# pasensio97/SDslam

Hardware: AMD Instinct MI355X
Metric: tracked frames/sec (ORB+ImageAlign+PnP) at 640x480, 1000 kp (higher is better)
Workload: dtype u8; 1 GPU; BASELINE configs[3] at the configs[1] pyramid: 640x480, 8-level x1.2, 1000 kp; ORB extract + ImageAlign (levels 4,3,2) + SearchByProjection + PnP RANSAC (maxIts 200; iterations actually run: tracking.mean_pnp_iterations with --full); pose_solver=pnp, pyramid=8x1.2, unique_scenes=64, inputs=resident in HBM, pose_records=packed on the device every step (single GPU: no collective)

## Files before the change

include/sdslam_hip.h:

```cpp
#ifndef SDSLAM_HIP_H_
#define SDSLAM_HIP_H_

#include <stddef.h>
#include <stdint.h>

#ifdef __cplusplus
extern "C" {
#endif

#define SD_OK 0
#define SD_ERR_INVALID_ARG 1
#define SD_ERR_HIP 2
#define SD_ERR_CAPACITY 3
#define SD_ERR_NO_DEVICE 4
#define SD_FALSE 100

const char* sd_last_error(void);
int sd_device_count(void);
const char* sd_version(void);

int sd_set_option(const char* name, int value);
int sd_get_option(const char* name, int* value);
int sd_option_count(void);
const char* sd_option_name(int index);
// ... 171 lines not shown
#define SD_REFRESH_NORMAL 2
#define SD_REFRESH_SKIPPED 16
#define SD_REFRESH_NOT_RESIDENT 32
#define SD_REFRESH_TOO_MANY 64
#define SD_REFRESH_BAD_INDEX 128
int sd_track_set_observations(sd_track* h, int n_points, const int32_t* obs_off, const int32_t* obs_frame, const int32_t* obs_kp,
                              const uint8_t* obs_kf_bad, const int32_t* ref_obs, const uint8_t* point_bad);
int sd_track_refresh_points(sd_track* h, int point_row, int write_local);
int sd_track_get_refreshed(sd_track* h, uint8_t* status, int32_t* best_obs, int32_t* best_median, uint8_t* desc, double* normal,
                           float* max_dist, float* min_dist, int cap);
int sd_debug_refresh_points(int n_points, const int32_t* obs_off, const uint8_t* obs_desc, const double* obs_centre,
                            const int32_t* obs_octave, const uint8_t* obs_kf_bad, const int32_t* ref_obs, const uint8_t* point_bad,
                            const double* Xw, const float* scale_factors, int nlevels, uint8_t* status, int32_t* best_obs,
                            int32_t* best_median, uint8_t* desc, double* normal, float* max_dist, float* min_dist);

int sd_track_align(sd_track* h, int n_frames, int mode);
int sd_track_match(sd_track* h, int n_frames, float th, int mono, int check_ori);
int sd_track_pnp(sd_track* h, int n_frames, double probability, int min_inliers, int max_iterations,
                 int min_set, float epsilon, float th2, int n_iterations);
int sd_track_pnp_iterate(sd_track* h, int n_frames, int n_iterations);
int sd_track_set_matches(sd_track* h, int frame0, int n_frames, const int32_t* cur_match, int cap);

int sd_track_get_align(sd_track* h, int frame0, int n_frames, double* Tcur_cm, double* error,
                       int32_t* ok, int32_t* iters, double* chi2);
int sd_track_get_matches(sd_track* h, int frame0, int n_frames, int32_t* cur_match, int cap,
                         int32_t* n_matches);
int sd_track_get_pnp(sd_track* h, int frame0, int n_frames, float* Tcw_rowmajor, uint8_t* inliers,
                     int cap, int32_t* info8);
int sd_debug_pnp_prof(unsigned long long* out32, int reset);
int sd_debug_align_prof(unsigned long long* out16, int reset);
int sd_debug_sel_prof(unsigned long long* out64, int reset);
int sd_debug_epnp(int n, const double* Xw, const double* uv, double fx, double fy, double cx, double cy,
                  double* R9, double* t3, double* reproj_err);
int sd_track_debug_read(sd_track* h, int which, int frame, void* out, size_t bytes);
int sd_track_debug_features_in_area(sd_track* h, int frame, float x, float y, float r, int min_level, int max_level,
                                    int32_t* indices, int cap, int32_t* n_out, int32_t* grid_counts);
int sd_track_pack_records(sd_track* h, int n_frames, int source, void* d_records);

int sd_track_set_map_ids(sd_track* h, int frame0, int n_frames, int which, const int32_t* ids, int cap);
int sd_track_advance(sd_track* h, int n_frames, int source);
int sd_track_set_prior(sd_track* h, int frame0, int n_frames, const double* T_cm, int relative);
int sd_track_get_last(sd_track* h, int frame0, int n_frames, int32_t* n_last, uint8_t* valid, double* Xw, uint8_t* desc, int32_t* octave,
                      float* angle, int32_t* obs, int32_t* ids);
int sd_track_get_extractors(sd_track* h, sd_orb** cur, sd_orb** ref);
int sd_track_close_points(sd_track* h, int n_frames, int source, float th_depth);
int sd_track_get_close_points(sd_track* h, int frame0, int n_frames, int32_t* out2);

int sd_track_motion_predict(sd_track* h, int n_frames, double dt);
int sd_track_motion_update(sd_track* h, int n_frames, int source);
int sd_track_motion_restart(sd_track* h, int frame0, int n_frames);
int sd_track_get_motion(sd_track* h, int frame0, int n_frames, double* X6, double* Pdiag6, int32_t* started, double* it_time,
                        double* E_cm, double* last_pose_cm);
int sd_track_set_motion(sd_track* h, int frame0, int n_frames, const double* X6, const double* Pdiag6, const int32_t* started,
                        const double* it_time);

#define SD_SENSOR_CONSTANT_VELOCITY 0
#define SD_SENSOR_IMU 1
int sd_track_set_sensor_model(sd_track* h, int model);
int sd_track_get_sensor_model(sd_track* h, int* model);
int sd_track_set_measurements(sd_track* h, int frame0, int n_frames, const double* wa6);
int sd_track_get_imu(sd_track* h, int frame0, int n_frames, double* X16, double* P256, double* gravity3, int32_t* started, double* it_time,
                     double* last_pose_cm, double* measurements6);
int sd_track_set_imu(sd_track* h, int frame0, int n_frames, const double* X16, const double* P256, const double* gravity3,
                     const int32_t* started, const double* it_time);
int sd_track_stream_fence(sd_track* h, void* hip_stream, int direction);
int sd_track_set_profiling(sd_track* h, int on);
// ... 19 lines not shown
```

sdslam_amd/capi.py:

```python
import ctypes as C
import os

import numpy as np

_HERE = os.path.dirname(os.path.abspath(__file__))
KP_DTYPE = np.dtype([("x", "<f4"), ("y", "<f4"), ("size", "<f4"), ("angle", "<f4"),
                     ("response", "<f4"), ("octave", "<i4"), ("class_id", "<i4")])
assert KP_DTYPE.itemsize == 28

SD_OK = 0


class SdError(RuntimeError):
    def __init__(self, code, msg):
        super().__init__(f"sdslam_hip status {code}: {msg}")
        self.code = code


def lib_path() -> str:
    return os.environ.get("SD_LIB") or os.path.join(_HERE, "libsdslam_hip.so")


_I, _F, _D, _Z, _P, _S = C.c_int, C.c_float, C.c_double, C.c_size_t, C.c_void_p, C.c_char_p
_PP, _PI = C.POINTER(C.c_void_p), C.POINTER(C.c_int)
# ... 71 lines not shown
    "sd_track_set_f12": (_I, [_P, _I, _I, _P]),
    "sd_track_search_for_triangulation": (_I, [_P, _I, _I, _I]),
    "sd_track_get_triangulation_matches": (_I, [_P, _I, _I, _P, _I, _P, _P, _P]),
    "sd_debug_search_for_triangulation": (_I, [_I, _I, _P, _P, _P, _P, _P, _P, _P, _P, _P, _P, _P, _P, _I, _I, _P, _P]),
    "sd_track_set_tri_depth": (_I, [_P, _I, _I, _I, _P, _I]),
    "sd_track_set_tri_median_depth": (_I, [_P, _I, _I, _P]),
    "sd_track_triangulate": (_I, [_P, _I, _I]),
    "sd_track_get_triangulated": (_I, [_P, _I, _I, _P, _P, _P, _I, _P]),
    "sd_track_get_new_points": (_I, [_P, _P, _P, _P, _P, _P, _P, _P, _P, _P, _P, _I]),
    "sd_debug_triangulate": (_I, [_I, _I, _P, _P, _P, _P, _P, _P, _P, _P, _P, _P, _P, _P, _P, _P, _I, _F, _I, _F, _P, _P, _P]),
    "sd_track_append_new_points": (_I, [_P, _I, _I, _I]),
    "sd_track_get_appended": (_I, [_P, _I, _I, _P, _P, _P]),
    "sd_track_get_local_points": (_I, [_P, _I, _P, _P, _P, _P, _P, _P, _P, _P, _P, _I]),
    "sd_track_set_fuse_scw": (_I, [_P, _I, _I, _P]),
    "sd_track_fuse": (_I, [_P, _I, _I, _I, _F, _I]),
    "sd_track_get_fuse": (_I, [_P, _I, _I, _P, _P, _I, _P]),
    "sd_debug_fuse": (_I, [_I, _P, _P, _P, _I, _P, _P, _P, _P, _P, _P, _P, _P, _I, _P, _P, _P, _I, _F, _F, _I, _I, _P, _P, _P, _P]),
    "sd_track_set_observations": (_I, [_P, _I, _P, _P, _P, _P, _P, _P]),
    "sd_track_refresh_points": (_I, [_P, _I, _I]),
    "sd_track_get_refreshed": (_I, [_P, _P, _P, _P, _P, _P, _P, _P, _I]),
    "sd_debug_refresh_points": (_I, [_I, _P, _P, _P, _P, _P, _P, _P, _P, _P, _I, _P, _P, _P, _P, _P, _P, _P]),
    "sd_track_align": (_I, [_P, _I, _I]),
    "sd_track_match": (_I, [_P, _I, _F, _I, _I]),
    "sd_track_pnp": (_I, [_P, _I, _D, _I, _I, _I, _F, _F, _I]),
    "sd_track_pnp_iterate": (_I, [_P, _I, _I]),
    "sd_track_set_matches": (_I, [_P, _I, _I, _P, _I]),
    "sd_track_get_align": (_I, [_P, _I, _I, _P, _P, _P, _P, _P]),
    "sd_track_get_matches": (_I, [_P, _I, _I, _P, _I, _P]),
    "sd_track_get_pnp": (_I, [_P, _I, _I, _P, _P, _I, _P]),
    "sd_debug_pnp_prof": (_I, [_P, _I]),
    "sd_debug_align_prof": (_I, [_P, _I]),
    "sd_debug_sel_prof": (_I, [_P, _I]),
    "sd_debug_epnp": (_I, [_I, _P, _P, _D, _D, _D, _D, _P, _P, _P]),
    "sd_track_debug_read": (_I, [_P, _I, _I, _P, _Z]),
    "sd_track_debug_features_in_area": (_I, [_P, _I, _F, _F, _F, _I, _I, _P, _I, _P, _P]),
    "sd_track_pack_records": (_I, [_P, _I, _I, _P]),
    "sd_track_set_map_ids": (_I, [_P, _I, _I, _I, _P, _I]),
    "sd_track_advance": (_I, [_P, _I, _I]),
    "sd_track_set_prior": (_I, [_P, _I, _I, _P, _I]),
    "sd_track_get_last": (_I, [_P, _I, _I, _P, _P, _P, _P, _P, _P, _P, _P]),
    "sd_track_get_extractors": (_I, [_P, _PP, _PP]),
    "sd_track_close_points": (_I, [_P, _I, _I, _F]),
    "sd_track_get_close_points": (_I, [_P, _I, _I, _P]),
    "sd_track_motion_predict": (_I, [_P, _I, _D]),
    "sd_track_motion_update": (_I, [_P, _I, _I]),
    "sd_track_motion_restart": (_I, [_P, _I, _I]),
    "sd_track_get_motion": (_I, [_P, _I, _I, _P, _P, _P, _P, _P, _P]),
    "sd_track_set_motion": (_I, [_P, _I, _I, _P, _P, _P, _P]),
    "sd_track_set_sensor_model": (_I, [_P, _I]),
    "sd_track_get_sensor_model": (_I, [_P, _PI]),
    "sd_track_set_measurements": (_I, [_P, _I, _I, _P]),
    "sd_track_get_imu": (_I, [_P, _I, _I, _P, _P, _P, _P, _P, _P, _P]),
    "sd_track_set_imu": (_I, [_P, _I, _I, _P, _P, _P, _P, _P]),
    "sd_track_stream_fence": (_I, [_P, _P, _I]),
    "sd_track_set_profiling": (_I, [_P, _I]),
    "sd_track_stage_ms": (_I, [_P, _P, _I]),
    "sd_track_set_next_map_id": (_I, [_P, _I, _I, _P]),
    "sd_track_stereo_init": (_I, [_P, _I, _I]),
    "sd_track_set_keyframe_state": (_I, [_P, _I, _I, _P]),
    "sd_track_need_keyframe": (_I, [_P, _I, _I, _I, _I, _I]),
    "sd_track_set_keyframe_flags": (_I, [_P, _I, _I, _P]),
    "sd_track_get_keyframe_flags": (_I, [_P, _I, _I, _P]),
    "sd_track_create_keyframe_points": (_I, [_P, _I, _I, _F, _I, _I]),
    "sd_track_get_created": (_I, [_P, _I, _I, _P, _P, _P, _P, _I]),
    "sd_hamming": (_I, [_P, _P]),
}
# ... 734 lines not shown
        _check(self.L.sd_track_get_keyframe_flags(self.h, frame0, n, _p(out)))
        return out

    def create_keyframe_points(self, n_frames, source, th_depth, use_flags=False, frame_id=0):
        _check(self.L.sd_track_create_keyframe_points(self.h, n_frames, int(source), float(th_depth), int(bool(use_flags)), int(frame_id)))

    def get_created(self, frame0, n, cap=None):
        cap = self.cap if cap is None else cap
        info = np.zeros((n, 4), np.int32)
        idx, ids, Xw = np.full((n, cap), -1, np.int32), np.full((n, cap), -1, np.int32), np.zeros((n, cap, 3))
        _check(self.L.sd_track_get_created(self.h, frame0, n, _p(info), _p(idx), _p(Xw), _p(ids), cap))
        return dict(mode=info[:, 0].copy(), created=info[:, 1].copy(), P=info[:, 2].copy(), candidates=info[:, 3].copy(), kp_index=idx,
                    Xw=Xw, ids=ids)

    def set_profiling(self, on=True):
        _check(self.L.sd_track_set_profiling(self.h, int(on)))

    def stage_ms(self):
        ms = np.zeros(3, np.float32)
        _check(self.L.sd_track_stage_ms(self.h, _p(ms), 3))
        return ms


def debug_epnp(Xw, uv, K):
    L = lib()
    Xw = np.ascontiguousarray(Xw, np.float64)
    uv = np.ascontiguousarray(uv, np.float64)
    R, t, e = np.zeros(9), np.zeros(3), C.c_double()
    _check(L.sd_debug_epnp(len(Xw), _p(Xw), _p(uv), float(K[0]), float(K[1]), float(K[2]), float(K[3]), _p(R), _p(t),
                           C.byref(e)))
    return R.reshape(3, 3), t, e.value


def debug_search_for_triangulation(kps1, desc1, has_mp1, uright1, kps2, desc2, has_mp2, uright2, F12, epipole, scale_factors,
                                   level_sigma2, check_ori=False):
    L = lib()
    k1, k2 = np.ascontiguousarray(kps1, KP_DTYPE), np.ascontiguousarray(kps2, KP_DTYPE)
    n1, n2 = len(k1), len(k2)
    d1, d2 = np.ascontiguousarray(desc1, np.uint8).reshape(n1, 32), np.ascontiguousarray(desc2, np.uint8).reshape(n2, 32)
    h1, h2 = np.ascontiguousarray(has_mp1, np.uint8), np.ascontiguousarray(has_mp2, np.uint8)
    u1, u2 = np.ascontiguousarray(uright1, np.float32), np.ascontiguousarray(uright2, np.float32)
    assert len(h1) == len(u1) == n1 and len(h2) == len(u2) == n2
    F, e = np.ascontiguousarray(F12, np.float64).reshape(9), np.ascontiguousarray(epipole, np.float32).reshape(2)
    sf, s2 = np.ascontiguousarray(scale_factors, np.float32), np.ascontiguousarray(level_sigma2, np.float32)
    assert len(sf) == len(s2)
    m, n = np.full(max(n1, 1), -1, np.int32), np.zeros(1, np.int32)
    _check(L.sd_debug_search_for_triangulation(n1, n2, _p(k1), _p(d1), _p(h1), _p(u1), _p(k2), _p(d2), _p(h2), _p(u2), _p(F), _p(e),
                                               _p(sf), _p(s2), len(sf), int(check_ori), _p(m), _p(n)))
    return int(n[0]), m[:n1]


def debug_triangulate(kps1_un, kps1, uright1, depth1, kps2_un, kps2, uright2, depth2, matches12, Tcw1, Tcw2, cam5, scale_factors,
                      level_sigma2, scale_factor, monocular=True, median_depth=-1.0):
    L = lib()
    k1u, k1 = np.ascontiguousarray(kps1_un, KP_DTYPE), np.ascontiguousarray(kps1, KP_DTYPE)
    k2u, k2 = np.ascontiguousarray(kps2_un, KP_DTYPE), np.ascontiguousarray(kps2, KP_DTYPE)
    n1, n2 = len(k1u), len(k2u)
    u1, z1 = np.ascontiguousarray(uright1, np.float32), np.ascontiguousarray(depth1, np.float32)
    u2, z2 = np.ascontiguousarray(uright2, np.float32), np.ascontiguousarray(depth2, np.float32)
    m = np.ascontiguousarray(matches12, np.int32)
    assert len(k1) == len(u1) == len(z1) == len(m) == n1 and len(k2) == len(u2) == len(z2) == n2
    T1, T2 = _cm(Tcw1), _cm(Tcw2)
    cam = np.ascontiguousarray(cam5, np.float32)
    sf, s2 = np.ascontiguousarray(scale_factors, np.float32), np.ascontiguousarray(level_sigma2, np.float32)
    assert len(cam) == 5 and len(sf) == len(s2)
    v, b, X = np.zeros(max(n1, 1), np.uint8), np.zeros(max(n1, 1), np.uint8), np.zeros((max(n1, 1), 3))
# ... 70 lines not shown
```

sdslam_amd/csrc/track.hip:

```cpp
#include <hip/hip_runtime.h>

#include <cmath>
#include <cstdlib>
#include <cstring>
#include <string>
#include <type_traits>
#include <vector>

#include "track_handle.h"

using namespace sd;

__global__ void k_pack_records(TrackBuffers tb, int source, int n_frames, double* __restrict__ out) {
  const int f = blockIdx.x * blockDim.x + threadIdx.x;
  if (f >= n_frames) return;
  double* r = out + (size_t)f * 20;
  if (source == 0) {
    const float* T = tb.pnp_T + (size_t)f * 16;
    for (int c = 0; c < 4; c++)
      for (int rr = 0; rr < 4; rr++) r[c * 4 + rr] = (double)T[rr * 4 + c];
  } else {
    const double* T = (source == 4 ? tb.Tcur : tb.po_T) + (size_t)f * 16;
    for (int i = 0; i < 16; i++) r[i] = T[i];
  }
// ... 755 lines not shown
}

int sd_track_get_pnp(sd_track* h, int frame0, int n_frames, float* Tcw_rowmajor, uint8_t* inliers, int cap, int32_t* info8) {
  TRACK_RANGE(h, frame0, n_frames);
  SD_REQUIRE(!inliers || cap >= h->kp_cap, SD_ERR_CAPACITY, "cap smaller than the keypoint capacity");
  hipStream_t s = h->cur->stream;
  SD_TRY(download(Tcw_rowmajor, h->tb.pnp_T, frame0, n_frames, 16, s));
  SD_TRY(download_rows(inliers, cap, h->tb.pnp_inliers, frame0, n_frames, h->kp_cap, s));
  SD_TRY(download(info8, h->tb.pnp_info, frame0, n_frames, 8, s));
  return wait_for(s);
}

int sd_debug_pnp_prof(unsigned long long* out32, int reset) {
  SD_REQUIRE(out32, SD_ERR_INVALID_ARG, "null output");
  return read_pnp_prof(out32, reset);
}

int sd_debug_sel_prof(unsigned long long* out64, int reset) {
  SD_REQUIRE(out64, SD_ERR_INVALID_ARG, "null output");
  return read_sel_prof(out64, reset);
}

int sd_debug_align_prof(unsigned long long* out16, int reset) {
  SD_REQUIRE(out16, SD_ERR_INVALID_ARG, "null output");
  return read_align_prof(out16, reset);
}

int sd_debug_epnp(int n, const double* Xw, const double* uv, double fx, double fy, double cx, double cy, double* R9, double* t3,
                  double* reproj_err) {
  SD_REQUIRE(n >= 4 && Xw && uv && R9 && t3, SD_ERR_INVALID_ARG, "bad arguments");
  return run_epnp_debug(n, Xw, uv, fx, fy, cx, cy, R9, t3, reproj_err);
}

int sd_track_debug_read(sd_track* h, int which, int frame, void* out, size_t bytes) {
  SD_REQUIRE(h && out && frame >= 0 && frame < h->max_batch, SD_ERR_INVALID_ARG, "bad arguments");
  SD_REQUIRE(which != 2 || bytes <= 15 * sizeof(double), SD_ERR_CAPACITY, "the Fuse pose of a slot is 15 doubles");
  const size_t M = (size_t)h->max_points, row = (size_t)frame * M;
  const size_t lm_bytes[5] = {M * 32, M * 24, M * 4, M * 4, M * 4};
  SD_REQUIRE(which < 3 || (which <= 7 && bytes <= lm_bytes[which - 3]), SD_ERR_CAPACITY, "unknown buffer or more bytes than a local-map row holds");
  SD_HIP_CHECK(hipSetDevice(h->device));
  SD_HIP_CHECK(hipStreamSynchronize(h->pnp_stream));
  SD_HIP_CHECK(hipStreamSynchronize(h->cur->stream));
  const void* src = which == 0   ? (const void*)(h->tb.pnp_pts + (size_t)frame * h->kp_cap * 6)
                    : which == 2 ? (const void*)(h->fu.pose + (size_t)frame * 15)
                    : which == 3 ? (const void*)(h->tb.lm_desc + row * 32)
                    : which == 4 ? (const void*)(h->tb.lm_normal + row * 3)
                    : which == 5 ? (const void*)(h->tb.lm_min + row)
                    : which == 6 ? (const void*)(h->tb.lm_max + row)
                    : which == 7 ? (const void*)(h->tb.lm_mfmax + row)
                                 : (const void*)(h->tb.pnp_kpidx + (size_t)frame * h->kp_cap);
  SD_HIP_CHECK(hipMemcpy(out, src, bytes, hipMemcpyDeviceToHost));
  return SD_OK;
}

int sd_track_debug_features_in_area(sd_track* h, int frame, float x, float y, float r, int min_level, int max_level, int32_t* indices,
                                    int cap, int32_t* n_out, int32_t* grid_counts) {
  SD_TRY(check_ready(h, frame + 1, true));
  SD_REQUIRE(frame >= 0 && indices && n_out && cap >= 0, SD_ERR_INVALID_ARG, "bad arguments");
  hipStream_t s = h->pnp_stream;
  SD_TRY(wait_inputs(h, false));
  int32_t* d = nullptr;
  const size_t n_ints = (size_t)h->kp_cap + 1 + 64 * 48;
  SD_HIP_CHECK(hipMalloc(&d, n_ints * sizeof(int32_t)));
  const int rc = launch_features_in_area(h->cur, h->tb, h->cam, frame, x, y, r, min_level, max_level, d, h->kp_cap, d + h->kp_cap, d + h->kp_cap + 1, s);
  std::vector<int32_t> host(n_ints);
  hipError_t e = hipMemcpyAsync(host.data(), d, n_ints * sizeof(int32_t), hipMemcpyDeviceToHost, s);
// ... 71 lines not shown
```

sdslam_amd/csrc/track_internal.h:

```cpp
#pragma once
#include <hip/hip_runtime.h>
#include <stdint.h>

#include "orb_internal.h"

namespace sd {

struct TrackBuffers {
  int max_points;
  int kp_cap;
  int cur_bcast;
  uint8_t* valid;
  double* Xw;
  uint8_t* mp_desc;
  int32_t* octave;
  float* angle;
  int32_t* obs;
  int32_t* n_last;
  int32_t* last_id;
  uint8_t* valid2;
  double* Xw2;
  uint8_t* mp_desc2;
  int32_t* octave2;
  float* angle2;
// ... 214 lines not shown
int launch_stereo_from_depth(const sd_orb* cur, const TrackBuffers& tb, const TrackCam& cam, const float* d_depth, int w, int h,
                             int stride_elems, size_t frame_stride_elems, int n_frames, hipStream_t s);
int launch_stereo_from_depth_typed(const sd_orb* cur, const TrackBuffers& tb, const TrackCam& cam, const void* d_depth, int u16,
                                   int convert, float scale, int w, int h, int stride_elems, size_t frame_stride_elems, int n_frames,
                                   hipStream_t s);
int launch_new_points(const sd_orb* cur, const TrackBuffers& tb, const TrackCam& cam, float inv_fx, float inv_fy, int n_frames, int mode,
                      int source, float th_depth, int use_flags, int frame_id, int min_keypoints, hipStream_t s);
int launch_need_keyframe(const TrackBuffers& tb, const int32_t* d_close, int n_frames, int rgbd, int frame_id, int min_frames,
                         int max_frames, hipStream_t s);
int launch_set_keyframe_state(const TrackBuffers& tb, const int32_t* staged, int frame0, int n_frames, hipStream_t s);
int launch_motion_init(const TrackBuffers& tb, int frame0, int n_frames, hipStream_t s);
int launch_motion_predict(const TrackBuffers& tb, int n_frames, double dt, hipStream_t s);
int launch_motion_update(const TrackBuffers& tb, int n_frames, int source, hipStream_t s);
int launch_imu_init(const TrackBuffers& tb, int frame0, int n_frames, int full, hipStream_t s);
int launch_imu_predict(const TrackBuffers& tb, int n_frames, double dt, hipStream_t s);
int launch_imu_update(const TrackBuffers& tb, int n_frames, int source, hipStream_t s);
int read_pnp_prof(unsigned long long* out32, int reset);
int read_sel_prof(unsigned long long* out64, int reset);
int read_align_prof(unsigned long long* out16, int reset);
int launch_pnp(const sd_orb* cur, const TrackBuffers& tb, const TrackCam& cam, const float* d_sigma2, const PnpParams& pp,
               int n_frames, hipStream_t s);

struct Sim3Params {
  int fix_scale, min_inliers;
  int n_iterations;
  int rand_per_frame;
  int resume;
};
int launch_sim3(const sd_orb* cur, const sd_orb* ref, const TrackBuffers& tb, const TrackCam& cam, const float* d_sigma2,
                const int32_t* d_max_its, const Sim3Params& sp, int n_frames, hipStream_t s);

int run_epnp_debug(int n, const double* Xw, const double* uv, double fx, double fy, double cx, double cy, double* R9, double* t3,
                   double* err);

}
```

sdslam_amd/csrc/track_pnp.hip:

```cpp
#include <hip/hip_runtime.h>

#include <algorithm>
#include <cfloat>
#include <cstdlib>

#include "orb_internal.h"
#include "sd_hypot.h"
#include "sd_wave.h"
#include "track_internal.h"
#include "track_pnp_lds.h"

namespace sd {

#define PNP_MAXN 2048
#define PNP_WORDS (PNP_MAXN / 64)
#define PNP_MAXSET 64

#ifdef SD_PNP_PROF
__device__ unsigned long long g_pnp_prof[32];
#define PROF_DECL long long _pt = clock64()
#define PROF(i)                                                                                       \
  do {                                                                                                \
    long long _n = clock64();                                                                         \
    if ((threadIdx.x & 63) == 0) atomicAdd(&g_pnp_prof[i], (unsigned long long)(_n - _pt));           \
    _pt = _n;                                                                                         \
  } while (0)
#else
#define PROF_DECL
#define PROF(i)
#endif

#ifndef PNP_FN
#define PNP_FN static __noinline__ __attribute__((disable_tail_calls))
#endif

typedef __attribute__((address_space(3))) double ldsd;
#define LDS_PTR(shared_array) ((ldsd*)(shared_array))
struct LArr {
  ldsd* p;
  __device__ __forceinline__ ldsd& operator[](int i) const { return p[i * PNP_CHUNK]; }
// ... 109 lines not shown
    for (int k = 0; k < m; k++) {
      double t = At[i * astep + k];
      sd += t * t;
    }
    sd = sqrt(sd);
  }
  *rng_io = rng;
  return sd;
}

template <int M, int N>
__device__ __forceinline__ void jacobi_svd_small(double (&At)[N][M], double (&Wout)[N], double (&Vt)[N][N]) {
  const double eps = DBL_EPSILON * 10, minval = DBL_MIN;
  double W[N];
#pragma unroll
  for (int i = 0; i < N; i++) {
    double sd = 0;
#pragma unroll
    for (int k = 0; k < M; k++) sd += At[i][k] * At[i][k];
    W[i] = sd;
#pragma unroll
    for (int k = 0; k < N; k++) Vt[i][k] = k == i ? 1 : 0;
  }
  for (int iter = 0; iter < 30; iter++) {
    bool changed = false;
#pragma unroll
    for (int i = 0; i < N - 1; i++) {
#pragma unroll
      for (int j = i + 1; j < N; j++) {
        double p = 0;
#pragma unroll
        for (int k = 0; k < M; k++) p += At[i][k] * At[j][k];
        if (!(fabs(p) <= eps * sqrt(W[i] * W[j]))) {
          p *= 2;
          double c, s;
          const double beta = W[i] - W[j], gamma = sdsc::hypot_glibc(p, beta);
          if (beta < 0) {
            const double delta = (gamma - beta) * 0.5;
            s = sqrt(delta / gamma);
            c = p / (gamma * s * 2);
          } else {
            c = sqrt((gamma + beta) / (gamma * 2));
            s = p / (gamma * c * 2);
          }
          double na = 0, nb = 0;
#pragma unroll
          for (int k = 0; k < M; k++) {
            const double t0 = c * At[i][k] + s * At[j][k];
            const double t1 = -s * At[i][k] + c * At[j][k];
            At[i][k] = t0;
            At[j][k] = t1;
            na += t0 * t0;
            nb += t1 * t1;
          }
          W[i] = na;
          W[j] = nb;
          changed = true;
#pragma unroll
          for (int k = 0; k < N; k++) {
            const double t0 = c * Vt[i][k] + s * Vt[j][k];
            const double t1 = -s * Vt[i][k] + c * Vt[j][k];
            Vt[i][k] = t0;
            Vt[j][k] = t1;
          }
        }
      }
    }
    if (!changed) break;
  }
#pragma unroll
  for (int i = 0; i < N; i++) {
    double sd = 0;
#pragma unroll
    for (int k = 0; k < M; k++) sd += At[i][k] * At[i][k];
    W[i] = sqrt(sd);
  }
#pragma unroll
// ... 20 lines not shown
  for (int i = 0; i < N; i++) Wout[i] = W[i];
  unsigned long long rng = 0x12345678ull;
#pragma unroll
  for (int i = 0; i < N; i++) {
    double sd = W[i];
    if (sd <= minval) {
      double tmp[N * M];
      for (int r = 0; r < N; r++)
        for (int k = 0; k < M; k++) tmp[r * M + k] = At[r][k];
      sd = jacobi_fill_row(tmp, M, M, i, &rng, sd);
#pragma unroll
      for (int k = 0; k < M; k++) At[i][k] = tmp[i * M + k];
    }
    const double s = sd > minval ? 1 / sd : 0.;
#pragma unroll
    for (int k = 0; k < M; k++) At[i][k] *= s;
  }
}

__device__ __forceinline__ bool jacobi_pair12(LMat A, int i, int j) {
  const double eps = DBL_EPSILON * 10;
  const LArr Ai = A.row(i), Aj = A.row(j);
  double ai[12], aj[12];
#pragma unroll
  for (int k = 0; k < 12; k++) {
    ai[k] = Ai[k];
    aj[k] = Aj[k];
  }
  double p = 0;
#pragma unroll
  for (int k = 0; k < 12; k++) p += ai[k] * aj[k];
  const double a = Ai[pnp_lds::kMatW], b = Aj[pnp_lds::kMatW];
  if (fabs(p) <= eps * sqrt(a * b)) return false;
  p *= 2;
  double c, s;
  const double beta = a - b, gamma = sdsc::hypot_glibc(p, beta);
  if (beta < 0) {
    const double delta = (gamma - beta) * 0.5;
    s = sqrt(delta / gamma);
    c = p / (gamma * s * 2);
  } else {
    c = sqrt((gamma + beta) / (gamma * 2));
    s = p / (gamma * c * 2);
  }
  double na = 0, nb = 0;
#pragma unroll
  for (int k = 0; k < 12; k++) {
    const double t0 = c * ai[k] + s * aj[k];
    const double t1 = -s * ai[k] + c * aj[k];
    Ai[k] = t0;
    Aj[k] = t1;
    na += t0 * t0;
    nb += t1 * t1;
  }
  Ai[pnp_lds::kMatW] = na;
  Aj[pnp_lds::kMatW] = nb;
  return true;
}

__device__ PNP_FN void jacobi_sweeps12_coop(LMat A, int g, bool act, unsigned long long group_mask) {
  if (act && g < 6)
    for (int i = g; i < 12; i += 6) {
      const LArr Ai = A.row(i);
      double sd = 0;
#pragma unroll
      for (int k = 0; k < 12; k++) {
        const double t = Ai[k];
        sd += t * t;
      }
      A.w(i) = sd;
    }
  __syncthreads();
  bool live = act;
  for (int iter = 0; iter < 30; iter++) {
    bool changed = false;
    for (int st = 1; st <= 21; st++) {
      const int i = max(0, st - 11) + g, j = st - i;
// ... 22 lines not shown
      Vt[i * 3 + j] = vt[i][j];
    }
  }
}

template <typename Ptr>
__device__ __forceinline__ void solve_svd6_n(int N, Ptr L, const int (&col)[5], const double (&b)[6], double (&x)[5]) {
  constexpr int M = 6, NM = 5;
  const double eps = DBL_EPSILON * 10, minval = DBL_MIN;
  double At[NM][M], Vt[NM][NM], W[NM];
#pragma unroll
  for (int i = 0; i < NM; i++) {
#pragma unroll
    for (int j = 0; j < M; j++) At[i][j] = i < N ? L[10 * j + col[i]] : 0.0;
    double sd = 0;
#pragma unroll
    for (int k = 0; k < M; k++) sd += At[i][k] * At[i][k];
    W[i] = sd;
#pragma unroll
    for (int k = 0; k < NM; k++) Vt[i][k] = k == i ? 1 : 0;
  }
  bool live = true;
  for (int iter = 0; iter < 30; iter++) {
    bool changed = false;
#pragma unroll
    for (int i = 0; i < NM - 1; i++) {
#pragma unroll
      for (int j = i + 1; j < NM; j++) {
        if (live && j < N) {
          double p = 0;
#pragma unroll
          for (int k = 0; k < M; k++) p += At[i][k] * At[j][k];
          if (!(fabs(p) <= eps * sqrt(W[i] * W[j]))) {
            p *= 2;
            double c, sn;
            const double beta = W[i] - W[j], gamma = sdsc::hypot_glibc(p, beta);
            if (beta < 0) {
              const double delta = (gamma - beta) * 0.5;
              sn = sqrt(delta / gamma);
              c = p / (gamma * sn * 2);
            } else {
              c = sqrt((gamma + beta) / (gamma * 2));
              sn = p / (gamma * c * 2);
            }
            double na = 0, nb = 0;
#pragma unroll
            for (int k = 0; k < M; k++) {
              const double t0 = c * At[i][k] + sn * At[j][k];
              const double t1 = -sn * At[i][k] + c * At[j][k];
              At[i][k] = t0;
              At[j][k] = t1;
              na += t0 * t0;
              nb += t1 * t1;
            }
            W[i] = na;
            W[j] = nb;
            changed = true;
#pragma unroll
            for (int k = 0; k < NM; k++) {
              const double t0 = c * Vt[i][k] + sn * Vt[j][k];
              const double t1 = -sn * Vt[i][k] + c * Vt[j][k];
              Vt[i][k] = t0;
              Vt[j][k] = t1;
            }
          }
        }
      }
    }
    live = live && changed;
    if (!__any(live)) break;
  }
#pragma unroll
  for (int i = 0; i < NM; i++) {
    double sd = 0;
#pragma unroll
    for (int k = 0; k < M; k++) sd += At[i][k] * At[i][k];
    W[i] = sqrt(sd);
// ... 431 lines not shown
    PROF(7);
    double sum2 = 0.0;
    for (int i = 0; i < n; i++) sum2 += epnp_reproj_term(Rv, tv, pws + 3 * i, us[2 * i], us[2 * i + 1], cam);
    err = sum2 / n;
    PROF(8);
  }
  return err;
}

template <int K, typename F>
__device__ __forceinline__ void ordered_sums(int n, ldsd* terms, ldsd* out, F&& term) {
  constexpr int KP = K | 1;
  const int lane = threadIdx.x & 63;
  double acc = 0;
  for (int base = 0; base < n; base += 64) {
    const int i = base + lane;
    if (i < n) {
      double tv[K];
      term(i, tv);
#pragma unroll
      for (int k = 0; k < K; k++) terms[lane * KP + k] = tv[k];
    }
    __syncthreads();
    const int cnt = min(64, n - base);
    if (lane < K) {
#pragma unroll 8
      for (int j = 0; j < cnt; j++) acc += terms[j * KP + lane];
    }
    __syncthreads();
  }
  if (lane < K) out[lane] = acc;
  __syncthreads();
}

template <typename TIn>
__device__ PNP_FN void epnp_refit_wave(int n, const TIn* pws, const TIn* us, const EpnpCam cam, ldsd* Rt_out, LMat ut, ldsd* scr) {
  const int lane = threadIdx.x & 63;
  ldsd* const terms = scr + pnp_lds::kTerms;
  ldsd* const mtm = scr + pnp_lds::kMtm;
  ldsd* const red = scr + pnp_lds::kRed;
  const LArr L{scr + pnp_lds::kRefitL};
  double cws[4][3], ci[9];
  auto PW = [&](int i, double* p) {
    p[0] = (double)pws[3 * i];
    p[1] = (double)pws[3 * i + 1];
    p[2] = (double)pws[3 * i + 2];
  };
  PROF_DECL;
  ordered_sums<3>(n, terms, red, [&](int i, double* tv) { PW(i, tv); });
  for (int j = 0; j < 3; j++) cws[0][j] = red[j] / n;
  ordered_sums<6>(n, terms, red, [&](int i, double* tv) {
    double pw[3];
    PW(i, pw);
    const double d0 = pw[0] - cws[0][0], d1 = pw[1] - cws[0][1], d2 = pw[2] - cws[0][2];
    tv[0] = d0 * d0; tv[1] = d0 * d1; tv[2] = d0 * d2;
    tv[3] = d1 * d1; tv[4] = d1 * d2; tv[5] = d2 * d2;
  });
  if (lane == 0) {
    const double pw0tpw0[9] = {red[0], red[1], red[2], red[1], red[3], red[4], red[2], red[4], red[5]};
    epnp_control_points(pw0tpw0, n, cws);
    epnp_cc_inverse(cws, ci);
    for (int i = 0; i < 9; i++) {
      red[16 + i] = cws[1 + i / 3][i % 3];
      red[32 + i] = ci[i];
    }
    for (int j = 0; j < 3; j++) red[48 + j] = cws[0][j];
// ... 46 lines not shown
          const double m2a = aa * (ca == 1 ? cam.fv : row[5]), m2b = ab * (cb == 1 ? cam.fv : row[5]);
          acc += has1 ? m1a * m1b : 0.0;
          acc += has2 ? m2a * m2b : 0.0;
        }
      }
    }
    if (mine) {
      mtm[ea * 12 + eb] = acc;
      mtm[eb * 12 + ea] = acc;
    }
  }
  __syncthreads();
  PROF(18);
  double rho[6];
  for (int i = lane; i < 144; i += 64) ut.row(i / 12)[i % 12] = mtm[i];
  __syncthreads();
  jacobi_sweeps12_coop(ut, lane, true, 0x3full);
  if (lane == 0) jacobi_finish12(ut);
  PROF(19);
  epnp_L_rho(ut, cws, L, rho, lane == 0);
  __syncthreads();
  PROF(20);
  if (lane < 3) {
    Rho6 rv;
    for (int i = 0; i < 6; i++) rv.r[i] = rho[i];
    Betas4 bt;
    epnp_betas(lane + 1, L, rv, bt);
    for (int i = 0; i < 4; i++) red[4 * lane + i] = bt.b[i];
  }
  __syncthreads();
  asm volatile("" ::: "memory");
  for (int i = 0; i < 12; i++) cws[i / 3][i % 3] = red[i < 3 ? 48 + i : 13 + i];
  for (int i = 0; i < 9; i++) ci[i] = red[32 + i];
  double betas3[3][4];
  for (int i = 0; i < 12; i++) betas3[i / 4][i % 4] = red[i];
  __syncthreads();
  PROF(22);
  double bestR[3][3], bestT[3], best_err = 0;
  for (int variant = 1; variant <= 3; variant++) {
    double ccs[4][3];
    epnp_ccs(ut, betas3[variant - 1], ccs);
    bool flip = false;
    auto PC = [&](int i, double* pc) {
      double a[4];
      AL(i, a);
      for (int j = 0; j < 3; j++) {
        const double x = a[0] * ccs[0][j] + a[1] * ccs[1][j] + a[2] * ccs[2][j] + a[3] * ccs[3][j];
        pc[j] = flip ? -x : x;
      }
    };
    {
      double pc_first[3];
      PC(0, pc_first);
      flip = pc_first[2] < 0.0;
    }
    double pc0[3], pw0[3], Rv[3][3], tv[3];
    ordered_sums<6>(n, terms, red, [&](int i, double* t6) {
      PC(i, t6);
      PW(i, t6 + 3);
    });
    for (int j = 0; j < 3; j++) {
      pc0[j] = red[j] / n;
      pw0[j] = red[3 + j] / n;
    }
    ordered_sums<9>(n, terms, red, [&](int i, double* t9) {
      double pc[3], pw[3];
      PC(i, pc);
      PW(i, pw);
      for (int j = 0; j < 3; j++) {
        t9[3 * j] = (pc[j] - pc0[j]) * (pw[0] - pw0[0]);
        t9[3 * j + 1] = (pc[j] - pc0[j]) * (pw[1] - pw0[1]);
        t9[3 * j + 2] = (pc[j] - pc0[j]) * (pw[2] - pw0[2]);
      }
    });
    if (lane == 0) {
      double abt[9];
      for (int i = 0; i < 9; i++) abt[i] = red[i];
      epnp_Rt_from_abt(abt, pc0, pw0, Rv, tv);
      for (int i = 0; i < 9; i++) red[16 + i] = Rv[i / 3][i % 3];
      for (int i = 0; i < 3; i++) red[25 + i] = tv[i];
    }
    __syncthreads();
    for (int i = 0; i < 9; i++) Rv[i / 3][i % 3] = red[16 + i];
    for (int i = 0; i < 3; i++) tv[i] = red[25 + i];
    PROF(23);
    ordered_sums<1>(n, terms, red, [&](int i, double* t1) {
      double pw[3];
      PW(i, pw);
      t1[0] = epnp_reproj_term(Rv, tv, pw, (double)us[2 * i], (double)us[2 * i + 1], cam);
    });
    const double err = red[0] / n;
    __syncthreads();
    PROF(24);
    if (variant == 1 || err < best_err) {
      best_err = err;
      for (int i = 0; i < 3; i++) {
        for (int j = 0; j < 3; j++) bestR[i][j] = Rv[i][j];
        bestT[i] = tv[i];
      }
    }
  }
  if (lane == 0) {
    for (int i = 0; i < 9; i++) Rt_out[i] = bestR[i / 3][i % 3];
    for (int i = 0; i < 3; i++) Rt_out[9 + i] = bestT[i];
    red[63] = best_err;
  }
  __syncthreads();
}

__device__ __forceinline__ bool pnp_is_inlier(const double* Rt, const float* q , const EpnpCam cam) {
  const float* p2 = q;
  const float* p3 = q + 2;
  const float maxErr = q[5];
  float Xc = (float)(Rt[0] * p3[0] + Rt[1] * p3[1] + Rt[2] * p3[2] + Rt[9]);
  float Yc = (float)(Rt[3] * p3[0] + Rt[4] * p3[1] + Rt[5] * p3[2] + Rt[10]);
  float invZc = (float)(1 / (Rt[6] * p3[0] + Rt[7] * p3[1] + Rt[8] * p3[2] + Rt[11]));
  double ue = cam.uc + cam.fu * Xc * invZc;
  double ve = cam.vc + cam.fv * Yc * invZc;
  float distX = (float)(p2[0] - ue);
  float distY = (float)(p2[1] - ve);
  float error2 = distX * distX + distY * distY;
  return error2 < maxErr;
}

template <bool kGeneral>
__global__ __launch_bounds__(64, 2) __attribute__((disable_tail_calls)) void k_pnp(const sd_keypoint* __restrict__ kps_all, const int32_t* __restrict__ nkp_all,
                                            TrackBuffers tb, TrackCam tcam, const float* __restrict__ sigma2, PnpParams pp,
                                            int n_frames) {
  __shared__ double s_work[pnp_lds::kWorkDoubles];
  __shared__ double s_Rt[PNP_CHUNK][12];
  __shared__ unsigned long long s_mask[PNP_CHUNK][PNP_WORDS];
  __shared__ unsigned long long s_best[PNP_WORDS], s_ref[PNP_WORDS];
  __shared__ int s_cnt[PNP_CHUNK];
  __shared__ double s_RtRef[12];
  __shared__ float s_bestT[12];
  __shared__ double s_scr[pnp_lds::kScrDoubles];
  __shared__ int s_modp[PNP_MAXSET], s_modv[PNP_MAXSET], s_draw[PNP_MAXSET];
  const int lane = threadIdx.x;
// ... 266 lines not shown
    for (int i = lane; i < N; i += 64)
      if ((s_ref[i >> 6] >> (i & 63)) & 1ull) inl_out[g_idx[i]] = 1;
    if (lane == 0) {
      for (int r = 0; r < 3; r++) {
        for (int c = 0; c < 3; c++) T_out[r * 4 + c] = (float)s_RtRef[r * 3 + c];
        T_out[r * 4 + 3] = (float)s_RtRef[9 + r];
      }
      T_out[12] = T_out[13] = T_out[14] = 0.f;
      T_out[15] = 1.f;
      info[0] = 1; info[1] = acc_cnt; info[2] = 0; info[3] = acc_iters; info[7] = 1;
    }
    return;
  }
  if (lane == 0) {
    info[2] = 1;
    info[3] = total;
  }
  if (best >= minInl) {
    for (int i = lane; i < N; i += 64)
      if ((s_best[i >> 6] >> (i & 63)) & 1ull) inl_out[g_idx[i]] = 1;
    if (lane == 0) {
      for (int r = 0; r < 3; r++) {
        for (int c = 0; c < 3; c++) T_out[r * 4 + c] = s_bestT[r * 3 + c];
        T_out[r * 4 + 3] = s_bestT[9 + r];
      }
      T_out[12] = T_out[13] = T_out[14] = 0.f;
      T_out[15] = 1.f;
      info[0] = 1;
      info[1] = best;
    }
  }
}

__global__ __launch_bounds__(64, 2) __attribute__((disable_tail_calls)) void k_epnp_debug(int n, const double* pws, const double* us, EpnpCam cam, double* out13) {
  __shared__ double s_work[pnp_lds::kWorkDoubles], s_scr[pnp_lds::kScrDoubles], s_Rt[12];
  const int lane = threadIdx.x;
  double e;
  if (n == 4) {
    double R[3][3], t[3];
    const int hyp = lane % PNP_CHUNK, variant = lane / PNP_CHUNK + 1;
    const bool active = hyp == 0 && variant <= 3;
    const LMat h_ut{LDS_PTR(s_work), hyp};
    const LArr h_L{LDS_PTR(s_scr) + pnp_lds::kL + hyp};
    const double err = epnp_minimal(
        active, variant,
        [&](int k, double* pw, double* u) {
          for (int j = 0; j < 3; j++) pw[j] = pws[3 * k + j];
          for (int j = 0; j < 2; j++) u[j] = us[2 * k + j];
        },
        cam, R, t, h_ut, h_L, LDS_PTR(s_scr), 1);
    const double e1 = __shfl(err, 0), e2 = __shfl(err, PNP_CHUNK), e3 = __shfl(err, 2 * PNP_CHUNK);
    int win = 1;
    e = e1;
    if (e2 < e) { win = 2; e = e2; }
    if (e3 < e) { win = 3; e = e3; }
    if (active && variant == win) {
      for (int i = 0; i < 9; i++) s_Rt[i] = R[i / 3][i % 3];
      for (int i = 0; i < 3; i++) s_Rt[9 + i] = t[i];
    }
    __syncthreads();
  } else {
    epnp_refit_wave(n, pws, us, cam, LDS_PTR(s_Rt), LMat{LDS_PTR(s_work), 0}, LDS_PTR(s_scr));
    e = s_scr[pnp_lds::kRed + 63];
  }
  if (lane == 0) {
    for (int i = 0; i < 12; i++) out13[i] = s_Rt[i];
    out13[12] = e;
  }
}

int run_epnp_debug(int n, const double* Xw, const double* uv, double fx, double fy, double cx, double cy, double* R9, double* t3,
                   double* err) {
  double *d_p = nullptr, *d_u = nullptr, *d_o = nullptr;
  SD_HIP_CHECK(hipMalloc(&d_p, sizeof(double) * 3 * n));
  SD_HIP_CHECK(hipMalloc(&d_u, sizeof(double) * 2 * n));
  SD_HIP_CHECK(hipMalloc(&d_o, sizeof(double) * 13));
  SD_HIP_CHECK(hipMemcpy(d_p, Xw, sizeof(double) * 3 * n, hipMemcpyHostToDevice));
  SD_HIP_CHECK(hipMemcpy(d_u, uv, sizeof(double) * 2 * n, hipMemcpyHostToDevice));
  EpnpCam cam = {fx, fy, cx, cy};
  hipLaunchKernelGGL(k_epnp_debug, dim3(1), dim3(64), 0, 0, n, d_p, d_u, cam, d_o);
  double out[13];
  SD_HIP_CHECK(hipMemcpy(out, d_o, sizeof(out), hipMemcpyDeviceToHost));
  for (int i = 0; i < 9; i++) R9[i] = out[i];
  for (int i = 0; i < 3; i++) t3[i] = out[9 + i];
  if (err) *err = out[12];
  (void)hipFree(d_p); (void)hipFree(d_u); (void)hipFree(d_o);
  return SD_OK;
}

int read_pnp_prof(unsigned long long* out32, int reset) {
#ifdef SD_PNP_PROF
  SD_HIP_CHECK(hipDeviceSynchronize());
  SD_HIP_CHECK(hipMemcpyFromSymbol(out32, HIP_SYMBOL(g_pnp_prof), 32 * sizeof(unsigned long long)));
  if (reset) {
    unsigned long long z[32] = {};
    SD_HIP_CHECK(hipMemcpyToSymbol(HIP_SYMBOL(g_pnp_prof), z, sizeof(z)));
  }
  return SD_OK;
#else
  set_error("library built without -DSD_PNP_PROF");
  return SD_ERR_INVALID_ARG;
#endif
}

int launch_pnp(const sd_orb* cur, const TrackBuffers& tb, const TrackCam& cam, const float* d_sigma2, const PnpParams& pp,
               int n_frames, hipStream_t s) {
  hipLaunchKernelGGL(pp.min_set == 4 ? k_pnp<false> : k_pnp<true>, dim3(n_frames), dim3(64), 0, s, keys_un(cur), cur->d_nout, tb, cam, d_sigma2, pp, n_frames);
  SD_HIP_CHECK(hipGetLastError());
  return SD_OK;
}

}
```

Measured before the change: 241,900 frames/s.

## Evaluate the three EPnP refit variants in parallel across wave lanes

Result: no change. 243,100 frames/s, median of 6 (+0.5%).

```diff
diff --git a/include/sdslam_hip.h b/include/sdslam_hip.h
--- a/include/sdslam_hip.h
+++ b/include/sdslam_hip.h
@@ -227,6 +227,8 @@
 int sd_debug_sel_prof(unsigned long long* out64, int reset);
 int sd_debug_epnp(int n, const double* Xw, const double* uv, double fx, double fy, double cx, double cy,
                   double* R9, double* t3, double* reproj_err);
+int sd_debug_epnp_variant(int n, const double* Xw, const double* uv, double fx, double fy, double cx, double cy,
+                          double* R9, double* t3, double* reproj_err, int32_t* variant2);
 int sd_track_debug_read(sd_track* h, int which, int frame, void* out, size_t bytes);
 int sd_track_debug_features_in_area(sd_track* h, int frame, float x, float y, float r, int min_level, int max_level,
                                     int32_t* indices, int cap, int32_t* n_out, int32_t* grid_counts);
diff --git a/sdslam_amd/capi.py b/sdslam_amd/capi.py
--- a/sdslam_amd/capi.py
+++ b/sdslam_amd/capi.py
@@ -127,6 +127,7 @@
     "sd_debug_align_prof": (_I, [_P, _I]),
     "sd_debug_sel_prof": (_I, [_P, _I]),
     "sd_debug_epnp": (_I, [_I, _P, _P, _D, _D, _D, _D, _P, _P, _P]),
+    "sd_debug_epnp_variant": (_I, [_I, _P, _P, _D, _D, _D, _D, _P, _P, _P, _P]),
     "sd_track_debug_read": (_I, [_P, _I, _I, _P, _Z]),
     "sd_track_debug_features_in_area": (_I, [_P, _I, _F, _F, _F, _I, _I, _P, _I, _P, _P]),
     "sd_track_pack_records": (_I, [_P, _I, _I, _P]),
@@ -927,6 +928,16 @@
     return R.reshape(3, 3), t, e.value
 
 
+def debug_epnp_variant(Xw, uv, K):
+    L = lib()
+    Xw = np.ascontiguousarray(Xw, np.float64)
+    uv = np.ascontiguousarray(uv, np.float64)
+    R, t, e, v = np.zeros(9), np.zeros(3), C.c_double(), np.zeros(2, np.int32)
+    _check(L.sd_debug_epnp_variant(len(Xw), _p(Xw), _p(uv), float(K[0]), float(K[1]), float(K[2]), float(K[3]), _p(R), _p(t),
+                                   C.byref(e), _p(v)))
+    return R.reshape(3, 3), t, e.value, int(v[0]), int(v[1])
+
+
 def debug_search_for_triangulation(kps1, desc1, has_mp1, uright1, kps2, desc2, has_mp2, uright2, F12, epipole, scale_factors,
                                    level_sigma2, check_ori=False):
     L = lib()
diff --git a/sdslam_amd/csrc/sd_jacobi_rot.h b/sdslam_amd/csrc/sd_jacobi_rot.h
--- /dev/null
+++ b/sdslam_amd/csrc/sd_jacobi_rot.h
@@ -0,0 +1,20 @@
+#pragma once
+#include <math.h>
+
+#include "sd_hypot.h"
+
+namespace sdsc {
+
+SD_HD void jacobi_rot(double p, double a, double b, double& c, double& s) {
+  p *= 2;
+  const double beta = a - b, gamma = hypot_glibc(p, beta);
+  const bool neg = beta < 0;
+  const double x = neg ? (gamma - beta) * 0.5 : gamma + beta;
+  const double y = neg ? gamma : gamma * 2;
+  const double r = sqrt(x / y);
+  const double o = p / (gamma * r * 2);
+  c = neg ? o : r;
+  s = neg ? r : o;
+}
+
+}
diff --git a/sdslam_amd/csrc/track.hip b/sdslam_amd/csrc/track.hip
--- a/sdslam_amd/csrc/track.hip
+++ b/sdslam_amd/csrc/track.hip
@@ -811,6 +811,12 @@
   return run_epnp_debug(n, Xw, uv, fx, fy, cx, cy, R9, t3, reproj_err);
 }
 
+int sd_debug_epnp_variant(int n, const double* Xw, const double* uv, double fx, double fy, double cx, double cy, double* R9, double* t3,
+                          double* reproj_err, int32_t* variant2) {
+  SD_REQUIRE(n >= 4 && Xw && uv && R9 && t3 && variant2, SD_ERR_INVALID_ARG, "bad arguments");
+  return run_epnp_debug_variant(n, Xw, uv, fx, fy, cx, cy, R9, t3, reproj_err, variant2);
+}
+
 int sd_track_debug_read(sd_track* h, int which, int frame, void* out, size_t bytes) {
   SD_REQUIRE(h && out && frame >= 0 && frame < h->max_batch, SD_ERR_INVALID_ARG, "bad arguments");
   SD_REQUIRE(which != 2 || bytes <= 15 * sizeof(double), SD_ERR_CAPACITY, "the Fuse pose of a slot is 15 doubles");
diff --git a/sdslam_amd/csrc/track_internal.h b/sdslam_amd/csrc/track_internal.h
--- a/sdslam_amd/csrc/track_internal.h
+++ b/sdslam_amd/csrc/track_internal.h
@@ -270,5 +270,7 @@
 
 int run_epnp_debug(int n, const double* Xw, const double* uv, double fx, double fy, double cx, double cy, double* R9, double* t3,
                    double* err);
-
-}
+int run_epnp_debug_variant(int n, const double* Xw, const double* uv, double fx, double fy, double cx, double cy, double* R9,
+                           double* t3, double* err, int32_t* variant2);
+
+}
diff --git a/sdslam_amd/csrc/track_pnp.hip b/sdslam_amd/csrc/track_pnp.hip
--- a/sdslam_amd/csrc/track_pnp.hip
+++ b/sdslam_amd/csrc/track_pnp.hip
@@ -6,6 +6,7 @@
 
 #include "orb_internal.h"
 #include "sd_hypot.h"
+#include "sd_jacobi_rot.h"
 #include "sd_wave.h"
 #include "track_internal.h"
 #include "track_pnp_lds.h"
@@ -181,17 +182,8 @@
 #pragma unroll
         for (int k = 0; k < M; k++) p += At[i][k] * At[j][k];
         if (!(fabs(p) <= eps * sqrt(W[i] * W[j]))) {
-          p *= 2;
           double c, s;
-          const double beta = W[i] - W[j], gamma = sdsc::hypot_glibc(p, beta);
-          if (beta < 0) {
-            const double delta = (gamma - beta) * 0.5;
-            s = sqrt(delta / gamma);
-            c = p / (gamma * s * 2);
-          } else {
-            c = sqrt((gamma + beta) / (gamma * 2));
-            s = p / (gamma * c * 2);
-          }
+          sdsc::jacobi_rot(p, W[i], W[j], c, s);
           double na = 0, nb = 0;
 #pragma unroll
           for (int k = 0; k < M; k++) {
@@ -278,17 +270,8 @@
   for (int k = 0; k < 12; k++) p += ai[k] * aj[k];
   const double a = Ai[pnp_lds::kMatW], b = Aj[pnp_lds::kMatW];
   if (fabs(p) <= eps * sqrt(a * b)) return false;
-  p *= 2;
   double c, s;
-  const double beta = a - b, gamma = sdsc::hypot_glibc(p, beta);
-  if (beta < 0) {
-    const double delta = (gamma - beta) * 0.5;
-    s = sqrt(delta / gamma);
-    c = p / (gamma * s * 2);
-  } else {
-    c = sqrt((gamma + beta) / (gamma * 2));
-    s = p / (gamma * c * 2);
-  }
+  sdsc::jacobi_rot(p, a, b, c, s);
   double na = 0, nb = 0;
 #pragma unroll
   for (int k = 0; k < 12; k++) {
@@ -377,17 +360,8 @@
 #pragma unroll
           for (int k = 0; k < M; k++) p += At[i][k] * At[j][k];
           if (!(fabs(p) <= eps * sqrt(W[i] * W[j]))) {
-            p *= 2;
             double c, sn;
-            const double beta = W[i] - W[j], gamma = sdsc::hypot_glibc(p, beta);
-            if (beta < 0) {
-              const double delta = (gamma - beta) * 0.5;
-              sn = sqrt(delta / gamma);
-              c = p / (gamma * sn * 2);
-            } else {
-              c = sqrt((gamma + beta) / (gamma * 2));
-              sn = p / (gamma * c * 2);
-            }
+            sdsc::jacobi_rot(p, W[i], W[j], c, sn);
             double na = 0, nb = 0;
 #pragma unroll
             for (int k = 0; k < M; k++) {
@@ -885,6 +859,34 @@
   if (lane < K) out[lane] = acc;
   __syncthreads();
 }
+
+template <int K, typename F>
+__device__ __forceinline__ void ordered_sums3(int n, ldsd* terms, ldsd* out, F&& term) {
+  constexpr int kBatch = 21;
+  static_assert(kBatch * 3 * 9 <= pnp_lds::kTermsSize && K <= 9, "a batch of terms fits the terms area");
+  const int lane = threadIdx.x & 63, il = lane / 3;
+  double acc = 0;
+  for (int base = 0; base < n; base += kBatch) {
+    const int i = base + il;
+    if (il < kBatch && i < n) {
+      double tv[K];
+      term(i, tv);
+#pragma unroll
+      for (int k = 0; k < K; k++) terms[lane * K + k] = tv[k];
+    }
+    __syncthreads();
+    const int cnt = min(kBatch, n - base);
+    if (lane < 3 * K) {
+#pragma unroll 7
+      for (int j = 0; j < cnt; j++) acc += terms[j * 3 * K + lane];
+    }
+    __syncthreads();
+  }
+  if (lane < 3 * K) out[lane] = acc;
+  __syncthreads();
+}
+
+constexpr int kRedWinner = 3, kRedFlip = 4, kRedErr = 63;
 
 template <typename TIn>
 __device__ PNP_FN void epnp_refit_wave(int n, const TIn* pws, const TIn* us, const EpnpCam cam, ldsd* Rt_out, LMat ut, ldsd* scr) {
@@ -997,78 +999,67 @@
   asm volatile("" ::: "memory");
   for (int i = 0; i < 12; i++) cws[i / 3][i % 3] = red[i < 3 ? 48 + i : 13 + i];
   for (int i = 0; i < 9; i++) ci[i] = red[32 + i];
-  double betas3[3][4];
-  for (int i = 0; i < 12; i++) betas3[i / 4][i % 4] = red[i];
+  const int v = lane % 3;
+  double betas[4];
+  for (int i = 0; i < 4; i++) betas[i] = red[4 * v + i];
   __syncthreads();
   PROF(22);
-  double bestR[3][3], bestT[3], best_err = 0;
-  for (int variant = 1; variant <= 3; variant++) {
-    double ccs[4][3];
-    epnp_ccs(ut, betas3[variant - 1], ccs);
-    bool flip = false;
-    auto PC = [&](int i, double* pc) {
-      double a[4];
-      AL(i, a);
-      for (int j = 0; j < 3; j++) {
-        const double x = a[0] * ccs[0][j] + a[1] * ccs[1][j] + a[2] * ccs[2][j] + a[3] * ccs[3][j];
-        pc[j] = flip ? -x : x;
-      }
-    };
-    {
-      double pc_first[3];
-      PC(0, pc_first);
-      flip = pc_first[2] < 0.0;
-    }
-    double pc0[3], pw0[3], Rv[3][3], tv[3];
-    ordered_sums<6>(n, terms, red, [&](int i, double* t6) {
-      PC(i, t6);
-      PW(i, t6 + 3);
-    });
+  constexpr int kRt3 = 27;
+  double ccs[4][3];
+  epnp_ccs(ut, betas, ccs);
+  bool flip = false;
+  auto PC = [&](int i, double* pc) {
+    double a[4];
+    AL(i, a);
     for (int j = 0; j < 3; j++) {
-      pc0[j] = red[j] / n;
-      pw0[j] = red[3 + j] / n;
-    }
-    ordered_sums<9>(n, terms, red, [&](int i, double* t9) {
-      double pc[3], pw[3];
-      PC(i, pc);
-      PW(i, pw);
-      for (int j = 0; j < 3; j++) {
-        t9[3 * j] = (pc[j] - pc0[j]) * (pw[0] - pw0[0]);
-        t9[3 * j + 1] = (pc[j] - pc0[j]) * (pw[1] - pw0[1]);
-        t9[3 * j + 2] = (pc[j] - pc0[j]) * (pw[2] - pw0[2]);
-      }
-    });
-    if (lane == 0) {
-      double abt[9];
-      for (int i = 0; i < 9; i++) abt[i] = red[i];
-      epnp_Rt_from_abt(abt, pc0, pw0, Rv, tv);
-      for (int i = 0; i < 9; i++) red[16 + i] = Rv[i / 3][i % 3];
-      for (int i = 0; i < 3; i++) red[25 + i] = tv[i];
-    }
-    __syncthreads();
-    for (int i = 0; i < 9; i++) Rv[i / 3][i % 3] = red[16 + i];
-    for (int i = 0; i < 3; i++) tv[i] = red[25 + i];
-    PROF(23);
-    ordered_sums<1>(n, terms, red, [&](int i, double* t1) {
-      double pw[3];
-      PW(i, pw);
-      t1[0] = epnp_reproj_term(Rv, tv, pw, (double)us[2 * i], (double)us[2 * i + 1], cam);
-    });
-    const double err = red[0] / n;
-    __syncthreads();
-    PROF(24);
-    if (variant == 1 || err < best_err) {
-      best_err = err;
-      for (int i = 0; i < 3; i++) {
-        for (int j = 0; j < 3; j++) bestR[i][j] = Rv[i][j];
-        bestT[i] = tv[i];
-      }
-    }
-  }
+      const double x = a[0] * ccs[0][j] + a[1] * ccs[1][j] + a[2] * ccs[2][j] + a[3] * ccs[3][j];
+      pc[j] = flip ? -x : x;
+    }
+  };
+  {
+    double pc_first[3];
+    PC(0, pc_first);
+    flip = pc_first[2] < 0.0;
+  }
+  double pc0[3], Rv[3][3], tv[3];
+  ordered_sums3<3>(n, terms, red, [&](int i, double* t3) { PC(i, t3); });
+  for (int j = 0; j < 3; j++) pc0[j] = red[3 * v + j] / n;
+  ordered_sums3<9>(n, terms, red, [&](int i, double* t9) {
+    double pc[3], pw[3];
+    PC(i, pc);
+    PW(i, pw);
+    for (int j = 0; j < 3; j++) {
+      t9[3 * j] = (pc[j] - pc0[j]) * (pw[0] - cws[0][0]);
+      t9[3 * j + 1] = (pc[j] - pc0[j]) * (pw[1] - cws[0][1]);
+      t9[3 * j + 2] = (pc[j] - pc0[j]) * (pw[2] - cws[0][2]);
+    }
+  });
+  if (lane < 3) {
+    double abt[9];
+    for (int i = 0; i < 9; i++) abt[i] = red[9 * lane + i];
+    epnp_Rt_from_abt(abt, pc0, cws[0], Rv, tv);
+    for (int i = 0; i < 9; i++) red[kRt3 + 12 * lane + i] = Rv[i / 3][i % 3];
+    for (int i = 0; i < 3; i++) red[kRt3 + 12 * lane + 9 + i] = tv[i];
+  }
+  __syncthreads();
+  for (int i = 0; i < 9; i++) Rv[i / 3][i % 3] = red[kRt3 + 12 * v + i];
+  for (int i = 0; i < 3; i++) tv[i] = red[kRt3 + 12 * v + 9 + i];
+  PROF(23);
+  ordered_sums3<1>(n, terms, red, [&](int i, double* t1) {
+    double pw[3];
+    PW(i, pw);
+    t1[0] = epnp_reproj_term(Rv, tv, pw, (double)us[2 * i], (double)us[2 * i + 1], cam);
+  });
+  PROF(24);
+  if (lane < 3) red[kRedFlip + lane] = flip ? 1.0 : 0.0;
   if (lane == 0) {
-    for (int i = 0; i < 9; i++) Rt_out[i] = bestR[i / 3][i % 3];
-    for (int i = 0; i < 3; i++) Rt_out[9 + i] = bestT[i];
-    red[63] = best_err;
+    const double e[4] = {0, red[0] / n, red[1] / n, red[2] / n};
+    int N = 1;
+    if (e[2] < e[1]) N = 2;
+    if (e[3] < e[N]) N = 3;
+    for (int i = 0; i < 12; i++) Rt_out[i] = red[kRt3 + 12 * (N - 1) + i];
+    red[kRedWinner] = (double)N;
+    red[kRedErr] = e[N];
   }
   __syncthreads();
 }
@@ -1401,10 +1392,11 @@
   }
 }
 
-__global__ __launch_bounds__(64, 2) __attribute__((disable_tail_calls)) void k_epnp_debug(int n, const double* pws, const double* us, EpnpCam cam, double* out13) {
+__global__ __launch_bounds__(64, 2) __attribute__((disable_tail_calls)) void k_epnp_debug(int n, const double* pws, const double* us, EpnpCam cam, double* out14) {
   __shared__ double s_work[pnp_lds::kWorkDoubles], s_scr[pnp_lds::kScrDoubles], s_Rt[12];
   const int lane = threadIdx.x;
   double e;
+  int win = 1, flips = 0;
   if (n == 4) {
     double R[3][3], t[3];
     const int hyp = lane % PNP_CHUNK, variant = lane / PNP_CHUNK + 1;
@@ -1419,7 +1411,6 @@
         },
         cam, R, t, h_ut, h_L, LDS_PTR(s_scr), 1);
     const double e1 = __shfl(err, 0), e2 = __shfl(err, PNP_CHUNK), e3 = __shfl(err, 2 * PNP_CHUNK);
-    int win = 1;
     e = e1;
     if (e2 < e) { win = 2; e = e2; }
     if (e3 < e) { win = 3; e = e3; }
@@ -1430,29 +1421,41 @@
     __syncthreads();
   } else {
     epnp_refit_wave(n, pws, us, cam, LDS_PTR(s_Rt), LMat{LDS_PTR(s_work), 0}, LDS_PTR(s_scr));
-    e = s_scr[pnp_lds::kRed + 63];
+    e = s_scr[pnp_lds::kRed + kRedErr];
+    win = (int)s_scr[pnp_lds::kRed + kRedWinner];
+    for (int k = 0; k < 3; k++) flips |= s_scr[pnp_lds::kRed + kRedFlip + k] != 0.0 ? 1 << k : 0;
   }
   if (lane == 0) {
-    for (int i = 0; i < 12; i++) out13[i] = s_Rt[i];
-    out13[12] = e;
+    for (int i = 0; i < 12; i++) out14[i] = s_Rt[i];
+    out14[12] = e;
+    out14[13] = (double)(win | flips << 8);
   }
 }
 
 int run_epnp_debug(int n, const double* Xw, const double* uv, double fx, double fy, double cx, double cy, double* R9, double* t3,
                    double* err) {
+  return run_epnp_debug_variant(n, Xw, uv, fx, fy, cx, cy, R9, t3, err, nullptr);
+}
+
+int run_epnp_debug_variant(int n, const double* Xw, const double* uv, double fx, double fy, double cx, double cy, double* R9,
+                           double* t3, double* err, int32_t* variant ) {
   double *d_p = nullptr, *d_u = nullptr, *d_o = nullptr;
   SD_HIP_CHECK(hipMalloc(&d_p, sizeof(double) * 3 * n));
   SD_HIP_CHECK(hipMalloc(&d_u, sizeof(double) * 2 * n));
-  SD_HIP_CHECK(hipMalloc(&d_o, sizeof(double) * 13));
+  SD_HIP_CHECK(hipMalloc(&d_o, sizeof(double) * 14));
   SD_HIP_CHECK(hipMemcpy(d_p, Xw, sizeof(double) * 3 * n, hipMemcpyHostToDevice));
   SD_HIP_CHECK(hipMemcpy(d_u, uv, sizeof(double) * 2 * n, hipMemcpyHostToDevice));
   EpnpCam cam = {fx, fy, cx, cy};
   hipLaunchKernelGGL(k_epnp_debug, dim3(1), dim3(64), 0, 0, n, d_p, d_u, cam, d_o);
-  double out[13];
+  double out[14];
   SD_HIP_CHECK(hipMemcpy(out, d_o, sizeof(out), hipMemcpyDeviceToHost));
   for (int i = 0; i < 9; i++) R9[i] = out[i];
   for (int i = 0; i < 3; i++) t3[i] = out[9 + i];
   if (err) *err = out[12];
+  if (variant) {
+    variant[0] = (int32_t)out[13] & 0xff;
+    variant[1] = (int32_t)out[13] >> 8;
+  }
   (void)hipFree(d_p); (void)hipFree(d_u); (void)hipFree(d_o);
   return SD_OK;
 }
```
